# Wangshihu12/colmap-pcd

Measured on AMD Instinct MI355X. Metric: NN queries/sec + BA-iter ms, 10M-pt cloud / 1M 3D feats, higher is better.
Workload: dtype f32 (NN distances) / f64 (association, BA); 1 GPU; M: 10000000-pt 'planes' cloud / 1000000 queries + BA scene 1000 cams / 1000000 pts / 4721253 obs / 900000 lidar terms (OPENCV), the same total at every N; cloud_points=10000000, queries=1000000, queries_this_rank=1000000, parallelism=single GPU

## Files before the change

### colmap-pcd_amd/csrc/ba.hip

```cpp
#include <algorithm>
#include <cmath>

#include "ba_cam_jac.h"
#include "ba_handle.h"
#include "ba_math.h"
#include "common.h"

namespace pcd {

template <int MODEL, bool SHARED>
struct BaCam {
  static constexpr int K = cam_num_params(MODEL >= 0 ? MODEL : 0);
  int model = MODEL;
  const double* p = nullptr;
  double v[K];
  __device__ __forceinline__ void resolve(const BaDev& d, int cm) {
    if (MODEL < 0) model = d.cam_model[cm];
    p = d.cam_params + d.cam_off[cm];
  }
  __device__ __forceinline__ explicit BaCam(const BaDev& d) {
    if (!SHARED) return;
    resolve(d, d.shared_cam);
    if (MODEL >= 0) {
#pragma unroll
      for (int k = 0; k < K; ++k) v[k] = p[k];
    }
  }
  __device__ __forceinline__ const double* params() const { return (SHARED && MODEL >= 0) ? v : p; }
  __device__ __forceinline__ void of_image(const BaDev& d, int im) {
    if (!SHARED) resolve(d, d.image_cam[im]);
  }
};

__device__ __forceinline__ void load_pose(const BaDev& d, int im, double pose[7]) {
#pragma unroll
  for (int k = 0; k < 7; ++k) pose[k] = d.poses[7 * (size_t)im + k];
}
template <int MODEL, bool SHARED>
__device__ __forceinline__ void eval_block_at(const BaCam<MODEL, SHARED>& cam, const double pose[7], const double X[3],
                                              double ox, double oy, ReprojBlock& b, double q[4]) {
  double t[3];
#pragma unroll
  for (int k = 0; k < 4; ++k) q[k] = pose[k];
#pragma unroll
  for (int k = 0; k < 3; ++k) t[k] = pose[4 + k];
  reproj_eval(cam.model, cam.params(), q, t, X, ox, oy, b);
}
template <int MODEL>
__device__ __forceinline__ void eval_block(const BaDev& d, int im, const double X[3], double ox, double oy,
                                           ReprojBlock& b, double q[4]) {
  const double* pose = d.poses + 7 * (size_t)im;
  double t[3];
#pragma unroll
  for (int k = 0; k < 4; ++k) q[k] = pose[k];
#pragma unroll
  for (int k = 0; k < 3; ++k) t[k] = pose[4 + k];
  const int cm = d.image_cam[im];
  const int model = MODEL >= 0 ? MODEL : d.cam_model[cm];
  reproj_eval(model, d.cam_params + d.cam_off[cm], q, t, X, ox, oy, b);
}
__device__ __forceinline__ double wave_uniform(double v) {
  const long long u = __double_as_longlong(v);
  const unsigned lo = (unsigned)__builtin_amdgcn_readfirstlane((int)(unsigned)u);
  const unsigned hi = (unsigned)__builtin_amdgcn_readfirstlane((int)(unsigned)((unsigned long long)u >> 32));
  return __longlong_as_double((long long)(((unsigned long long)hi << 32) | lo));
}

template <int N>
__device__ __forceinline__ void wave_store_rows(double* __restrict__ out, uint64_t row0, int cnt, const double (&v)[N],
                                                double* __restrict__ lds) {
  static_assert(N % 2 == 0, "rows are moved in 16-byte units");
  const int lane = threadIdx.x & 63;
#pragma unroll
  for (int k = 0; k < N; ++k) lds[lane * N + k] = v[k];
  __builtin_amdgcn_fence(__ATOMIC_RELEASE, "workgroup");
  __builtin_amdgcn_wave_barrier();
  __builtin_amdgcn_fence(__ATOMIC_ACQUIRE, "workgroup");
  const double2* src = reinterpret_cast<const double2*>(lds);
  double2* dst = reinterpret_cast<double2*>(out + row0 * N);
  const int units = cnt * (N / 2);
#pragma unroll
  for (int j = 0; j < N / 2; ++j) {
    const int u = j * 64 + lane;
    if (u < units) dst[u] = src[u];
  }
  __builtin_amdgcn_fence(__ATOMIC_RELEASE, "workgroup");
  __builtin_amdgcn_wave_barrier();
}

template <int MODEL, bool BLOCKS, bool SHARED>
__global__ __launch_bounds__(256) void k_ba_points(BaDev d, double* __restrict__ Hpt, double* __restrict__ gpt,
                                                   double* __restrict__ cost_partial) {
  __shared__ double s_half[2][64][9];
  const int sl = threadIdx.x >> 7, half = (threadIdx.x >> 6) & 1, lane = threadIdx.x & 63;
  const int slice = blockIdx.x * 2 + sl;
  const int t = slice * 64 + lane;
  double cost = 0.0;
  double H[6] = {0, 0, 0, 0, 0, 0}, g[3] = {0, 0, 0};
  int p = -1;
  bool cpt = true;
  double X[3] = {0, 0, 0};
  BaCam<MODEL, SHARED> cam(d);
  if (slice < d.nslices) {
    p = d.pt_order[t];
    const uint32_t s0 = d.slice_start[slice], s1 = d.slice_start[slice + 1];
    if (p >= 0) {
      X[0] = d.points[3 * (size_t)p]; X[1] = d.points[3 * (size_t)p + 1]; X[2] = d.points[3 * (size_t)p + 2];
      cpt = d.point_const && d.point_const[p];
    }
    for (uint32_t s = s0 + lane + 64u * half; s < s1; s += 128) {
      const int im = d.sell_img[s];
      if (im < 0) continue;
      ReprojBlock b;
      double q[4], pose[7];
      cam.of_image(d, im);
      load_pose(d, im, pose);
      eval_block_at(cam, pose, X, d.sell_xy[2 * (size_t)s], d.sell_xy[2 * (size_t)s + 1], b, q);
      double rho0, rho1;
      loss_eval(d.loss_type, d.loss_scale, b.r[0] * b.r[0] + b.r[1] * b.r[1], rho0, rho1);
      cost += 0.5 * rho0;
      if (BLOCKS && !cpt) {
        const double sr = sqrt(rho1);
        double J[6];
#pragma unroll
        for (int r = 0; r < 2; ++r)
#pragma unroll
          for (int k = 0; k < 3; ++k)
            J[3 * r + k] = sr * (b.M[3 * r] * b.D[k] + b.M[3 * r + 1] * b.D[3 + k] + b.M[3 * r + 2] * b.D[6 + k]);
        const double r0 = sr * b.r[0], r1 = sr * b.r[1];
        H[0] += J[0] * J[0] + J[3] * J[3]; H[1] += J[0] * J[1] + J[3] * J[4]; H[2] += J[0] * J[2] + J[3] * J[5];
        H[3] += J[1] * J[1] + J[4] * J[4]; H[4] += J[1] * J[2] + J[4] * J[5]; H[5] += J[2] * J[2] + J[5] * J[5];
        g[0] += J[0] * r0 + J[3] * r1; g[1] += J[1] * r0 + J[4] * r1; g[2] += J[2] * r0 + J[5] * r1;
      }
    }
  }
  if (BLOCKS && half == 1) {
#pragma unroll
    for (int k = 0; k < 6; ++k) s_half[sl][lane][k] = H[k];
#pragma unroll
    for (int k = 0; k < 3; ++k) s_half[sl][lane][6 + k] = g[k];
  }
  __syncthreads();
  if (half == 0 && slice < d.nslices) {
    if (BLOCKS) {
#pragma unroll
      for (int k = 0; k < 6; ++k) H[k] += s_half[sl][lane][k];
#pragma unroll
      for (int k = 0; k < 3; ++k) g[k] += s_half[sl][lane][6 + k];
    }
    if (p >= 0) {
      for (uint32_t e = d.pt_lidar_start[p]; e < d.pt_lidar_start[p + 1]; ++e) {
        const uint32_t l = d.pt_lidar_list[e];
        const double abcd[4] = {d.lidar_abcd[4 * (size_t)l], d.lidar_abcd[4 * (size_t)l + 1],
                                d.lidar_abcd[4 * (size_t)l + 2], d.lidar_abcd[4 * (size_t)l + 3]};
        double r, J[3];
        lidar_eval(X, abcd, d.lidar_w[l], 0, r, J);
        double rho0, rho1;
        loss_eval(d.loss_type, d.loss_scale, r * r, rho0, rho1);
        cost += 0.5 * rho0;
        if (BLOCKS && !cpt) {
          const double sr = sqrt(rho1);
          const double rc = sr * r;
          J[0] *= sr; J[1] *= sr; J[2] *= sr;
          H[0] += J[0] * J[0]; H[1] += J[0] * J[1]; H[2] += J[0] * J[2];
          H[3] += J[1] * J[1]; H[4] += J[1] * J[2]; H[5] += J[2] * J[2];
          g[0] += J[0] * rc; g[1] += J[1] * rc; g[2] += J[2] * rc;
        }
      }
      if (BLOCKS && Hpt) {
        double* h = Hpt + 9 * (size_t)p;
        h[0] = H[0]; h[1] = H[1]; h[2] = H[2]; h[3] = H[1]; h[4] = H[3]; h[5] = H[4]; h[6] = H[2]; h[7] = H[4]; h[8] = H[5];
      }
      if (BLOCKS && gpt) { gpt[3 * (size_t)p] = g[0]; gpt[3 * (size_t)p + 1] = g[1]; gpt[3 * (size_t)p + 2] = g[2]; }
    }
  }
  __syncthreads();
  __shared__ double s_c[256];
  s_c[threadIdx.x] = cost;
  __syncthreads();
  for (int off = 128; off > 0; off >>= 1) {
    if ((int)threadIdx.x < off) s_c[threadIdx.x] += s_c[threadIdx.x + off];
    __syncthreads();
  }
  if (threadIdx.x == 0) cost_partial[blockIdx.x] = s_c[0];
}

template <int MODEL, bool SHARED>
__global__ __launch_bounds__(256) void k_ba_cost(BaDev d, double* __restrict__ cost_partial) {
  double cost = 0.0;
  BaCam<MODEL, SHARED> cam(d);
  for (uint64_t i = blockIdx.x * (uint64_t)256 + threadIdx.x; i < d.O + d.L; i += (uint64_t)gridDim.x * 256) {
    if (i < d.O) {
      const int im = d.obs_image[i], pt = d.obs_point[i];
      const double X[3] = {d.points[3 * (size_t)pt], d.points[3 * (size_t)pt + 1], d.points[3 * (size_t)pt + 2]};
      ReprojBlock b;
      double q[4];
      double pose[7];
      const int im0 = __builtin_amdgcn_readfirstlane(im);
      if (__all(im == im0)) {
#pragma unroll
        for (int k = 0; k < 7; ++k) pose[k] = wave_uniform(d.poses[7 * (size_t)im0 + k]);
      } else {
        load_pose(d, im, pose);
      }
      cam.of_image(d, im);
      eval_block_at(cam, pose, X, d.obs_xy[2 * i], d.obs_xy[2 * i + 1], b, q);
      double rho0, rho1;
      loss_eval(d.loss_type, d.loss_scale, b.r[0] * b.r[0] + b.r[1] * b.r[1], rho0, rho1);
      cost += 0.5 * rho0;
    } else {
      const uint64_t l = i - d.O;
      const int pt = d.lidar_point[l];
      const double X[3] = {d.points[3 * (size_t)pt], d.points[3 * (size_t)pt + 1], d.points[3 * (size_t)pt + 2]};
      const double abcd[4] = {d.lidar_abcd[4 * l], d.lidar_abcd[4 * l + 1], d.lidar_abcd[4 * l + 2], d.lidar_abcd[4 * l + 3]};
      double r, J[3];
      lidar_eval(X, abcd, d.lidar_w[l], 0, r, J);
      double rho0, rho1;
      loss_eval(d.loss_type, d.loss_scale, r * r, rho0, rho1);
      cost += 0.5 * rho0;
    }
  }
  __shared__ double s_c[256];
  s_c[threadIdx.x] = cost;
  __syncthreads();
  for (int off = 128; off > 0; off >>= 1) {
    if ((int)threadIdx.x < off) s_c[threadIdx.x] += s_c[threadIdx.x + off];
    __syncthreads();
  }
  if (threadIdx.x == 0) cost_partial[blockIdx.x] = s_c[0];
}
constexpr unsigned kCostBlocks = 1u << 20;

constexpr int kSumThreads = 1024;
__global__ __launch_bounds__(kSumThreads) void k_sum_partials(const double* __restrict__ partial, int n,
                                                              double* __restrict__ out) {
  constexpr int T = kSumThreads;
  __shared__ double s_c[T];
  double a[8] = {0.0, 0.0, 0.0, 0.0, 0.0, 0.0, 0.0, 0.0};
  int i = threadIdx.x;
  for (; i + 7 * T < n; i += 8 * T) {
#pragma unroll
    for (int j = 0; j < 8; ++j) a[j] += partial[i + j * T];
  }
  for (; i < n; i += T) a[0] += partial[i];
  s_c[threadIdx.x] = ((a[0] + a[1]) + (a[2] + a[3])) + ((a[4] + a[5]) + (a[6] + a[7]));
  __syncthreads();
  for (int off = T / 2; off > 0; off >>= 1) {
    if ((int)threadIdx.x < off) s_c[threadIdx.x] += s_c[threadIdx.x + off];
    __syncthreads();
  }
  if (threadIdx.x == 0) out[0] = s_c[0];
}

constexpr uint32_t kImgSeg = 1024;
constexpr int kRowColStride = 132;
static_assert(7 * kRowColStride <= 64 * 18, "the staged rows share the W transpose scratch");
typedef double mfma_f64x4 __attribute__((ext_vector_type(4)));

template <int MODEL, bool WANT_W>
__global__ __launch_bounds__(256, (MODEL == 4 && WANT_W) ? 4 : 1) void k_ba_images(BaDev d, double* __restrict__ partial,
                                                                       double* __restrict__ W_o) {
  __shared__ __attribute__((aligned(16))) double s_w[4][64 * 18];
  __shared__ double s_a[4][2][27];
  const int im = (int)d.seg_img[blockIdx.x];
  const int lane = threadIdx.x & 63;
  const int wave = __builtin_amdgcn_readfirstlane((int)(threadIdx.x >> 6));
  const bool cpose = d.image_const_pose && d.image_const_pose[im];
  mfma_f64x4 acc = {0.0, 0.0, 0.0, 0.0};
  const unsigned tmask = d.image_const_tvec ? d.image_const_tvec[im] : 0u;
  const uint32_t e_beg = d.seg_begin[blockIdx.x];
  const uint32_t e_end = min(d.seg_begin[blockIdx.x + 1], d.img_obs_start[im + 1]);
  const int op_k = lane >> 4, op_c = (lane & 7) == 7 ? 0 : (lane & 7);
  const double* op_src = s_w[wave] + op_c * kRowColStride + 2 * op_k + ((lane >> 3) & 1);
  if (!cpose || WANT_W) {
    for (uint32_t e0 = e_beg; e0 < e_end; e0 += 256) {
      const uint32_t e = e0 + threadIdx.x;
      const bool active = e < e_end;
      const int cnt = (int)min(64u, e_end > e0 + wave * 64u ? e_end - (e0 + wave * 64u) : 0u);
      double w[18];
#pragma unroll
      for (int k = 0; k < 18; ++k) w[k] = 0.0;
      double J[12], r0 = 0.0, r1 = 0.0;
#pragma unroll
      for (int k = 0; k < 12; ++k) J[k] = 0.0;
      if (active && !cpose) {
        const int pt = d.img_pt[e];
        const double X[3] = {d.points[3 * (size_t)pt], d.points[3 * (size_t)pt + 1], d.points[3 * (size_t)pt + 2]};
        ReprojBlock b;
        double q[4];
        eval_block<MODEL>(d, im, X, d.img_xy[2 * (size_t)e], d.img_xy[2 * (size_t)e + 1], b, q);
        double rho0, rho1;
        loss_eval(d.loss_type, d.loss_scale, b.r[0] * b.r[0] + b.r[1] * b.r[1], rho0, rho1);
        const double sr = sqrt(rho1);
        double Jq[8], Jt[6], JX[6], Jqt[6];
        reproj_jacobians(b, Jq, Jt, JX);
        quat_tangent(q, Jq, Jqt);
#pragma unroll
        for (int r = 0; r < 2; ++r)
#pragma unroll
          for (int k = 0; k < 3; ++k) {
            J[6 * r + k] = sr * Jqt[3 * r + k];
            J[6 * r + 3 + k] = ((tmask >> k) & 1u) ? 0.0 : sr * Jt[3 * r + k];
          }
        r0 = sr * b.r[0];
        r1 = sr * b.r[1];
        if (WANT_W && !(d.point_const && d.point_const[pt])) {
#pragma unroll
          for (int a = 0; a < 6; ++a)
#pragma unroll
            for (int c = 0; c < 3; ++c) w[3 * a + c] = J[a] * (sr * JX[c]) + J[6 + a] * (sr * JX[3 + c]);
        }
      }
      if (!cpose && cnt > 0) {
        double2* row_dst = reinterpret_cast<double2*>(s_w[wave]) + lane;
#pragma unroll
        for (int c = 0; c < 6; ++c) row_dst[c * (kRowColStride / 2)] = make_double2(J[c], J[6 + c]);
        row_dst[6 * (kRowColStride / 2)] = make_double2(r0, r1);
        __builtin_amdgcn_fence(__ATOMIC_RELEASE, "workgroup");
        __builtin_amdgcn_wave_barrier();
        __builtin_amdgcn_fence(__ATOMIC_ACQUIRE, "workgroup");
#pragma unroll
        for (int s = 0; s < 16; ++s) {
          const double a = op_src[8 * s];
          acc = __builtin_amdgcn_mfma_f64_16x16x4f64(a, a, acc, 0, 0, 0);
        }
        __builtin_amdgcn_fence(__ATOMIC_RELEASE, "workgroup");
        __builtin_amdgcn_wave_barrier();
      }
      if (WANT_W) {
        const uint32_t o = active ? d.img_obs[e] : 0u;
        const uint32_t o_first = (uint32_t)__builtin_amdgcn_readfirstlane((int)o);
        const bool contiguous = __all(!active || o == o_first + (uint32_t)lane);
        if (contiguous) {
          wave_store_rows<18>(W_o, o_first, cnt, w, s_w[wave]);
        } else if (active) {
          double* dst = W_o + 18 * (size_t)o;
#pragma unroll
          for (int k = 0; k < 18; ++k) dst[k] = w[k];
        }
      }
    }
  }
  {
    const int g = lane >> 4, h = (lane >> 3) & 1, c = lane & 7;
#pragma unroll
    for (int hi = 0; hi < 2; ++hi) {
      const int a = g + 4 * hi;
      const double v = h ? acc[2 + hi] : acc[hi];
      if (a < 6 && c >= a && c < 7) s_a[wave][h][c == 6 ? 21 + a : a * 6 - a * (a - 1) / 2 + (c - a)] = v;
    }
  }
  __syncthreads();
  if (threadIdx.x < 27) {
    const int k = threadIdx.x;
    partial[27 * (size_t)blockIdx.x + k] = ((s_a[0][0][k] + s_a[0][1][k]) + (s_a[1][0][k] + s_a[1][1][k])) +
                                           ((s_a[2][0][k] + s_a[2][1][k]) + (s_a[3][0][k] + s_a[3][1][k]));
  }
}

__global__ __launch_bounds__(64) void k_ba_images_reduce(BaDev d, const double* __restrict__ partial,
                                                         double* __restrict__ Himg, double* __restrict__ gimg) {
  const int im = blockIdx.x * 2 + (threadIdx.x >> 5), k = threadIdx.x & 31;
  if (im >= d.I || k >= 27) return;
  double v = 0.0;
  for (uint32_t sgm = d.img_seg_start[im]; sgm < d.img_seg_start[im + 1]; ++sgm) v += partial[27 * (size_t)sgm + k];
  if (k >= 21) {
    if (gimg) gimg[6 * (size_t)im + (k - 21)] = v;
  } else if (Himg) {
    int a = 0, kk = k;
    while (kk >= 6 - a) { kk -= 6 - a; ++a; }
    const int c = a + kk;
    Himg[36 * (size_t)im + 6 * a + c] = v;
    Himg[36 * (size_t)im + 6 * c + a] = v;
  }
}

__host__ __device__ constexpr int cam_ne(int K) { return K * (K + 1) / 2 + 6 * K + K; }
__host__ __device__ constexpr int cam_ent_l(int K, int e) {
  const int ncc = K * (K + 1) / 2;
  if (e < ncc) { int a = 0; while (e >= K - a) { e -= K - a; ++a; } return a; }
  e -= ncc;
  if (e < 6 * K) return e / 6;
  return e - 6 * K;
}
__host__ __device__ constexpr int cam_ent_r(int K, int e) {
  const int ncc = K * (K + 1) / 2;
  if (e < ncc) { int a = 0; while (e >= K - a) { e -= K - a; ++a; } return a + e; }
  e -= ncc;
  if (e < 6 * K) return K + e % 6;
  return K + 6;
}

template <int MODEL, int CH>
__device__ __forceinline__ void cam_accumulate(const BaDev& d, int im, double* __restrict__ partial) {
  constexpr int K = MODEL >= 0 ? cam_num_params(MODEL >= 0 ? MODEL : 0) : PCD_CAM_JAC_STRIDE;
  constexpr int NE = cam_ne(K), PER = (NE + 3) / 4, E0 = CH * PER, E1 = E0 + PER < NE ? E0 + PER : NE;
  constexpr int NA = K + 7;
  const int lane = threadIdx.x & 63;
  const bool cpose = d.image_const_pose && d.image_const_pose[im];
  const unsigned tmask = d.image_const_tvec ? d.image_const_tvec[im] : 0u;
  const int cm = d.image_cam[im];
  const double* cam = d.cam_params + d.cam_off[cm];
  const uint8_t* refine = d.cam_refine ? d.cam_refine + d.cam_off[cm] : nullptr;
  const int model = MODEL >= 0 ? MODEL : d.cam_model[cm];
  double acc[PER > 0 ? PER : 1];
#pragma unroll
  for (int t = 0; t < PER; ++t) acc[t] = 0.0;
  for (uint32_t e = d.img_obs_start[im] + lane; e < d.img_obs_start[im + 1]; e += 64) {
    const int pt = d.img_pt[e];
    const double X[3] = {d.points[3 * (size_t)pt], d.points[3 * (size_t)pt + 1], d.points[3 * (size_t)pt + 2]};
    ReprojBlock b;
    double q[4];
    eval_block<MODEL>(d, im, X, d.img_xy[2 * (size_t)e], d.img_xy[2 * (size_t)e + 1], b, q);
    double rho0, rho1;
    loss_eval(d.loss_type, d.loss_scale, b.r[0] * b.r[0] + b.r[1] * b.r[1], rho0, rho1);
    const double sr = sqrt(rho1);
    double A[2][NA];
    {
      const double* pose = d.poses + 7 * (size_t)im;
// ... 508 lines not shown
}

static void launch_points(const pcd_ba* b, const BaDev& d, double* Hpt, double* gpt, hipStream_t s) {
  PCD_BA_DISPATCH_CAM(b->uniform_model, d.shared_cam >= 0,
                      hipLaunchKernelGGL((k_ba_points<M, true, SH>), dim3(cost_blocks(b, true)), dim3(256), 0, s, d, Hpt, gpt,
                                         b->cost_partial.p));
}
static void launch_images(const pcd_ba* b, const BaDev& d, double* Himg, double* gimg, double* W, hipStream_t s) {
  if (b->nseg) {
    PCD_BA_DISPATCH(b->uniform_model,
                    if (W) hipLaunchKernelGGL((k_ba_images<M, true>), dim3(b->nseg), dim3(256), 0, s, d, b->img_partial.p, W);
                    else hipLaunchKernelGGL((k_ba_images<M, false>), dim3(b->nseg), dim3(256), 0, s, d, b->img_partial.p, W));
  }
  hipLaunchKernelGGL(k_ba_images_reduce, dim3(div_up(b->I, 2)), dim3(64), 0, s, d, b->img_partial.p, Himg, gimg);
}

pcd_status pcd::ba_normal_equations(pcd_ba* b, const uint32_t* w_order, double* Hpt, double* gpt, double* cost,
                                    double* Himg, double* gimg, double* W, hipStream_t s) {
  PCD_TRY(b->img_partial.reserve(27 * (size_t)std::max(b->nseg, 1u)));
  BaDev d = b->dev();
  launch_points(b, d, Hpt, gpt, s);
  hipLaunchKernelGGL(k_sum_partials, dim3(1), dim3(kSumThreads), 0, s, b->cost_partial.p, (int)cost_blocks(b, true), cost);
  if (w_order) d.img_obs = w_order;
  launch_images(b, d, Himg, gimg, W, s);
  return PCD_OK;
}

extern "C" {

pcd_status pcd_ba_create(const pcd_ba_desc* d, pcd_ba** out) {
  return pcd::guard([&]() -> pcd_status {
  PCD_REQUIRE(d && out, "null pointer");
  *out = nullptr;
  PCD_REQUIRE(d->num_cameras > 0 && d->cam_model && d->cam_param_offset && d->cam_params, "cameras");
  PCD_REQUIRE(d->num_images > 0 && d->poses && d->image_camera, "images");
  PCD_REQUIRE(d->num_points > 0 && d->points, "points");
  PCD_REQUIRE(d->num_obs == 0 || (d->obs_image && d->obs_point && d->obs_xy), "observations");
  PCD_REQUIRE(d->num_lidar == 0 || (d->lidar_point && d->lidar_abcd && d->lidar_weight), "lidar terms");
  PCD_REQUIRE(d->loss_type >= 0 && d->loss_type <= 2, "loss_type");
  PCD_REQUIRE(d->loss_type == PCD_LOSS_TRIVIAL || d->loss_scale > 0, "loss_scale");
  PCD_REQUIRE(d->num_obs < 0xFFFFFFF0ull && d->num_lidar < 0xFFFFFFF0ull, "too many residual blocks");
  for (int c = 0; c < d->num_cameras; ++c) {
    const int k = pcd_camera_num_params(d->cam_model[c]);
    PCD_REQUIRE(k > 0, "unknown camera model id");
    PCD_REQUIRE(d->cam_param_offset[c] >= 0 && (uint64_t)d->cam_param_offset[c] + k <= d->cam_params_len,
                "camera parameter offsets");
  }
  for (int i = 0; i < d->num_images; ++i)
    PCD_REQUIRE(d->image_camera[i] >= 0 && d->image_camera[i] < d->num_cameras, "image_camera out of range");
  for (uint64_t o = 0; o < d->num_obs; ++o) {
    PCD_REQUIRE(d->obs_image[o] >= 0 && d->obs_image[o] < d->num_images, "obs_image out of range");
    PCD_REQUIRE(d->obs_point[o] >= 0 && d->obs_point[o] < d->num_points, "obs_point out of range");
  }
  for (uint64_t l = 0; l < d->num_lidar; ++l)
    PCD_REQUIRE(d->lidar_point[l] >= 0 && d->lidar_point[l] < d->num_points, "lidar_point out of range");
  PCD_TRY(require_device(d->device));

  pcd_ba* b = new pcd_ba();
  b->device = d->device;
  b->C = d->num_cameras; b->I = d->num_images; b->P = d->num_points; b->O = d->num_obs; b->L = d->num_lidar;
  b->loss_type = d->loss_type; b->loss_scale = d->loss_scale;
  b->cam_params_len = d->cam_params_len;
  for (int c = 0; c < d->num_cameras; ++c) b->cam_stride = std::max(b->cam_stride, cam_num_params(d->cam_model[c]));
  b->uniform_model = d->cam_model[0];
  for (int c = 1; c < d->num_cameras; ++c)
    if (d->cam_model[c] != b->uniform_model) b->uniform_model = -1;
  b->shared_cam = d->image_camera[0];
  for (int i = 1; i < d->num_images; ++i)
    if (d->image_camera[i] != b->shared_cam) b->shared_cam = -1;
  auto fail = [&](pcd_status st) { pcd_ba_destroy(b); return st; };
#define UP(buf, src, n) do { pcd_status _st = upload(b->buf, src, (size_t)(n)); if (_st != PCD_OK) return fail(_st); } while (0)
  UP(cam_model, d->cam_model, b->C); UP(cam_off, d->cam_param_offset, b->C); UP(cam_params, d->cam_params, d->cam_params_len);
  UP(poses, d->poses, 7 * (size_t)b->I); UP(image_cam, d->image_camera, b->I);
  UP(points, d->points, 3 * (size_t)b->P);
  UP(obs_image, d->obs_image, b->O); UP(obs_point, d->obs_point, b->O); UP(obs_xy, d->obs_xy, 2 * b->O);
  UP(lidar_point, d->lidar_point, b->L); UP(lidar_abcd, d->lidar_abcd, 4 * b->L); UP(lidar_w, d->lidar_weight, b->L);
  if (d->image_const_pose) { b->has_cpose = true; UP(image_const_pose, d->image_const_pose, b->I); }
  if (d->image_const_tvec) { b->has_ctvec = true; UP(image_const_tvec, d->image_const_tvec, b->I); }
  if (d->point_const) { b->has_cpt = true; UP(point_const, d->point_const, b->P); }
  if (d->camera_refine) { b->has_refine = true; UP(cam_refine, d->camera_refine, d->cam_params_len); }
  for (uint64_t k = 0; d->camera_refine && k < d->cam_params_len; ++k) b->refines_intrinsics |= d->camera_refine[k] != 0;

  std::vector<uint32_t> st, li;
  build_csr(d->obs_point, b->O, b->P, st, li);
  {
    uint32_t maxlen = 0;
    for (int p = 0; p < b->P; ++p) maxlen = std::max(maxlen, st[p + 1] - st[p]);
    std::vector<uint32_t> bucket((size_t)maxlen + 2, 0);
    for (int p = 0; p < b->P; ++p) bucket[(size_t)(st[p + 1] - st[p]) + 1]++;
    for (size_t k = 1; k < bucket.size(); ++k) bucket[k] += bucket[k - 1];
    const int nslices = (b->P + 63) / 64;
    b->nslices = nslices;
    std::vector<int> order((size_t)nslices * 64, -1);
    for (int p = 0; p < b->P; ++p) order[bucket[st[p + 1] - st[p]]++] = p;
    std::vector<uint32_t> slice_start(nslices + 1, 0);
    for (int s = 0; s < nslices; ++s) {
      uint32_t mx = 0;
      for (int l = 63; l >= 0; --l) {
        const int p = order[(size_t)s * 64 + l];
        if (p >= 0) { mx = st[p + 1] - st[p]; break; }
      }
      slice_start[s + 1] = slice_start[s] + mx * 64;
    }
    const size_t nslots = slice_start[nslices];
    UP(pt_order, order.data(), order.size());
    UP(slice_start, slice_start.data(), slice_start.size());
    UP(pt_obs_start, st.data(), st.size()); UP(pt_obs_list, li.data(), li.size());
    UP(pt_lidar_start, st.data(), st.size()); UP(pt_lidar_list, li.data(), li.size());
    pcd_status sa = b->sell_img.reserve(std::max<size_t>(nslots, 1));
    if (sa == PCD_OK) sa = b->sell_xy.reserve(std::max<size_t>(2 * nslots, 2));
    if (sa != PCD_OK) return fail(sa);
    if (nslots)
      hipLaunchKernelGGL(k_ba_fill_sell, dim3(div_up((size_t)nslices * 64, 256)), dim3(256), 0, nullptr, b->pt_order.p,
                         b->slice_start.p, b->pt_lidar_start.p, b->pt_lidar_list.p, b->obs_image.p, b->obs_xy.p, nslices,
                         b->sell_img.p, b->sell_xy.p);
    if (hipDeviceSynchronize() != hipSuccess || hipGetLastError() != hipSuccess) {
      set_error("pcd_ba_create: filling the per-track layout failed");
      return fail(PCD_ERR_HIP);
    }
  }
  build_csr(d->lidar_point, b->L, b->P, st, li);
  UP(pt_lidar_start, st.data(), st.size()); UP(pt_lidar_list, li.data(), li.size());
  build_csr(d->obs_image, b->O, b->I, st, li);
  {
    UP(img_obs_start, st.data(), st.size());
    {
      std::vector<uint32_t> seg_img, seg_begin, img_seg_start(b->I + 1, 0);
      for (int i = 0; i < b->I; ++i) {
        img_seg_start[i] = (uint32_t)seg_img.size();
        for (uint32_t e = st[i]; e < st[i + 1]; e += kImgSeg) { seg_img.push_back((uint32_t)i); seg_begin.push_back(e); }
      }
      img_seg_start[b->I] = (uint32_t)seg_img.size();
      b->nseg = (uint32_t)seg_img.size();
      seg_begin.push_back((uint32_t)b->O);
      UP(seg_img, seg_img.data(), seg_img.size());
      UP(seg_begin, seg_begin.data(), seg_begin.size());
      UP(img_seg_start, img_seg_start.data(), img_seg_start.size());
    }
    {
      std::vector<uint32_t> cst, cli;
      build_csr(d->image_camera, (uint64_t)b->I, b->C, cst, cli);
      UP(cam_img_start, cst.data(), cst.size());
      UP(cam_img_list, cli.data(), cli.size());
    }
    UP(img_obs, li.data(), li.size());
    pcd_status sa = b->img_pt.reserve(std::max<size_t>(b->O, 1));
    if (sa == PCD_OK) sa = b->img_xy.reserve(std::max<size_t>(2 * b->O, 2));
    if (sa != PCD_OK) return fail(sa);
    if (b->O)
      hipLaunchKernelGGL(k_ba_fill_image_major, dim3(div_up(b->O, 256)), dim3(256), 0, nullptr, b->img_obs.p,
                         b->obs_point.p, b->obs_xy.p, b->O, b->img_pt.p, b->img_xy.p);
    if (hipDeviceSynchronize() != hipSuccess || hipGetLastError() != hipSuccess) {
      set_error("pcd_ba_create: filling the image-major layout failed");
      return fail(PCD_ERR_HIP);
    }
  }
#undef UP
  {
    b->h_pose_row.assign(b->O, 0xFFFFFFFFu);
    std::vector<uint32_t> vobs;
    vobs.reserve(b->O);
    for (uint64_t o = 0; o < b->O; ++o)
      if (!(d->image_const_pose && d->image_const_pose[d->obs_image[o]])) {
        b->h_pose_row[o] = (uint32_t)vobs.size();
        vobs.push_back((uint32_t)o);
      }
    b->n_pose_rows = vobs.size();
    if (b->n_pose_rows != b->O) {
      pcd_status sv = upload(b->vobs, vobs.data(), vobs.size());
      if (sv != PCD_OK) return fail(sv);
    }
  }
  pcd_status s1 = b->cost_partial.reserve((size_t)std::max(cost_blocks(b, true), cost_blocks(b, false)) + 1);
  if (s1 != PCD_OK) return fail(s1);
  if ((s1 = b->cost.reserve(1)) != PCD_OK) return fail(s1);
  *out = b;
  return PCD_OK;
  });
}

void pcd_ba_destroy(pcd_ba* b) {
  if (!b) return;
  (void)hipSetDevice(b->device);
  delete b;
}

pcd_status pcd_ba_set_parameters(pcd_ba* b, const double* poses, const double* points) {
  PCD_REQUIRE(b, "null handle");
  PCD_HIP_TRY(hipSetDevice(b->device));
  if (poses) PCD_HIP_TRY(hipMemcpy(b->poses.p, poses, 7 * (size_t)b->I * sizeof(double), hipMemcpyHostToDevice));
  if (points) PCD_HIP_TRY(hipMemcpy(b->points.p, points, 3 * (size_t)b->P * sizeof(double), hipMemcpyHostToDevice));
  return PCD_OK;
}

pcd_status pcd_ba_set_parameters_device(pcd_ba* b, const double* d_poses, const double* d_points, void* stream) {
  PCD_TRY(require_device(b ? b->device : 0));
  PCD_REQUIRE(b, "null handle");
  PCD_REFUSE_CAPTURE(stream);
  PCD_HIP_TRY(hipSetDevice(b->device));
  hipStream_t s = (hipStream_t)stream;
  if (d_poses && d_poses != b->poses.p)
    PCD_HIP_TRY(hipMemcpyAsync(b->poses.p, d_poses, 7 * (size_t)b->I * sizeof(double), hipMemcpyDeviceToDevice, s));
  if (d_points && d_points != b->points.p)
    PCD_HIP_TRY(hipMemcpyAsync(b->points.p, d_points, 3 * (size_t)b->P * sizeof(double), hipMemcpyDeviceToDevice, s));
  return PCD_OK;
// ... 292 lines not shown
```

### colmap-pcd_amd/csrc/ba_handle.h

```cpp
#pragma once
#include <memory>

#include "ba_cam_jac.h"
#include "common.h"

namespace pcd {

struct BaDev {
  const int* cam_model; const int* cam_off; const double* cam_params;
  const double* poses; const int* image_cam; const uint8_t* image_const_pose; const uint8_t* image_const_tvec;
  const double* points; const uint8_t* point_const;
  const int* obs_image; const int* obs_point; const double* obs_xy;
  const int* lidar_point; const double* lidar_abcd; const double* lidar_w;
  const int* pt_order;
  const uint32_t* slice_start;
  const int* sell_img;
  const double* sell_xy;
  const uint32_t* pt_lidar_start; const uint32_t* pt_lidar_list;
  const uint32_t* img_obs_start;
  const int* img_pt;
  const uint32_t* img_obs;
  const uint32_t* seg_img;
  const uint32_t* seg_begin;
  const uint32_t* img_seg_start;
  const uint8_t* cam_refine;
  const uint32_t* cam_img_start;
  const uint32_t* cam_img_list;
  int C;
  int cam_k;
  const double* img_xy;
  int I, P, nslices; uint64_t O, L;
  int loss_type; double loss_scale;
  int shared_cam;
};

struct BaSchur;
struct BaSchurDelete { void operator()(BaSchur* s) const; };

template <typename T>
static pcd_status upload(DevBuf<T>& b, const T* src, size_t n) {
  PCD_TRY(b.reserve(std::max<size_t>(n, 1)));
  if (n) PCD_HIP_TRY(hipMemcpy(b.p, src, n * sizeof(T), hipMemcpyHostToDevice));
  return PCD_OK;
}

pcd_status ba_normal_equations(pcd_ba* b, const uint32_t* w_order, double* Hpt, double* gpt, double* cost, double* Himg,
                               double* gimg, double* W, hipStream_t s);

}

struct pcd_ba {
  int device = 0;
  int C = 0, I = 0, P = 0, nslices = 0;
  uint64_t O = 0, L = 0, cam_params_len = 0;
  int loss_type = 0;
  double loss_scale = 1.0;
  int uniform_model = -1;
  int shared_cam = -1;
  pcd::DevBuf<int> cam_model, cam_off, image_cam, obs_image, obs_point, lidar_point, pt_order, sell_img, img_pt;
  pcd::DevBuf<double> cam_params, poses, points, obs_xy, lidar_abcd, lidar_w, sell_xy, img_xy;
  pcd::DevBuf<uint8_t> image_const_pose, image_const_tvec, point_const;
  bool has_cpose = false, has_ctvec = false, has_cpt = false;
  pcd::DevBuf<uint32_t> slice_start, pt_lidar_start, pt_lidar_list, img_obs_start, img_obs, cam_img_start, cam_img_list;
  pcd::DevBuf<uint32_t> seg_img, seg_begin, img_seg_start;
  uint32_t nseg = 0;
  pcd::DevBuf<double> img_partial;
  pcd::DevBuf<uint8_t> cam_refine;
  bool has_refine = false;
  pcd::DevBuf<double> cam_partial;
  pcd::DevBuf<double> cost_partial, cost;
  pcd::DevBuf<double> o_res, o_jq, o_jt, o_jx, o_jl, o_himg, o_gimg, o_hpt, o_gpt, o_w, o_jc, o_hcam, o_gcam, o_ecam, o_wcam;
  std::vector<uint32_t> h_pose_row;
  uint64_t n_pose_rows = 0;
  pcd::DevBuf<uint32_t> vobs;
  pcd::DevBuf<double> p_jq, p_jt;
  pcd::PinnedBuf<double> h_blocks;
  int cam_stride = 0;
  pcd::DevBuf<double> o_rec, p_jc;
  pcd::DevBuf<uint32_t> pt_obs_start, pt_obs_list;
  pcd::DevBuf<double> f_sq, f_depth, f_part, f_summary;
  pcd::DevBuf<uint8_t> f_u8;
  bool refines_intrinsics = false;
  std::unique_ptr<pcd::BaSchur, pcd::BaSchurDelete> schur;
  pcd::BaDev dev() const {
    pcd::BaDev d;
    d.cam_model = cam_model.p; d.cam_off = cam_off.p; d.cam_params = cam_params.p;
    d.poses = poses.p; d.image_cam = image_cam.p;
    d.image_const_pose = has_cpose ? image_const_pose.p : nullptr;
    d.image_const_tvec = has_ctvec ? image_const_tvec.p : nullptr;
    d.points = points.p; d.point_const = has_cpt ? point_const.p : nullptr;
    d.obs_image = obs_image.p; d.obs_point = obs_point.p; d.obs_xy = obs_xy.p;
    d.lidar_point = lidar_point.p; d.lidar_abcd = lidar_abcd.p; d.lidar_w = lidar_w.p;
    d.pt_order = pt_order.p; d.slice_start = slice_start.p; d.sell_img = sell_img.p; d.sell_xy = sell_xy.p;
    d.pt_lidar_start = pt_lidar_start.p; d.pt_lidar_list = pt_lidar_list.p;
    d.img_obs_start = img_obs_start.p; d.img_pt = img_pt.p; d.img_xy = img_xy.p; d.img_obs = img_obs.p;
    d.seg_img = seg_img.p; d.seg_begin = seg_begin.p; d.img_seg_start = img_seg_start.p;
    d.cam_refine = has_refine ? cam_refine.p : nullptr; d.cam_img_start = cam_img_start.p; d.cam_img_list = cam_img_list.p;
    d.C = C; d.shared_cam = shared_cam; d.cam_k = (uniform_model >= 0 && uniform_model <= 4) ? pcd::cam_num_params(uniform_model) : PCD_CAM_JAC_STRIDE;
    d.I = I; d.P = P; d.nslices = nslices; d.O = O; d.L = L; d.loss_type = loss_type; d.loss_scale = loss_scale;
    return d;
  }
};
```

Before: 781.3 million queries/s.

## Prefetch BA point/image operands and precompute first lidar term per slot

In the points kernel, the next SELL image index and the observation xy are now software-prefetched one iteration ahead. The first lidar plane for each thread slot is precomputed on the host into a coalesced SoA array, which removes the dependent CSR indirection for the common single-term case. In the image kernel, camera parameters and pose are hoisted out of the loop as wave-uniform values pinned in SGPRs, and the next point index, coordinates and const flag are prefetched across iterations. This is meant to hide gather latency in BA, at the cost of extra device buffers, more registers and inline-asm register pinning that may hurt occupancy.

```diff
diff --git a/colmap-pcd_amd/csrc/ba.hip b/colmap-pcd_amd/csrc/ba.hip
--- a/colmap-pcd_amd/csrc/ba.hip
+++ b/colmap-pcd_amd/csrc/ba.hip
@@ -66,11 +66,21 @@
   return __longlong_as_double((long long)(((unsigned long long)hi << 32) | lo));
 }
 
+__device__ __forceinline__ double sgpr_pin(double v) {
+  asm volatile("" : "+s"(v));
+  return v;
+}
+
+template <typename T>
+__device__ __forceinline__ T vgpr_pin(T v) {
+  asm volatile("" : "+v"(v));
+  return v;
+}
+
 template <int N>
 __device__ __forceinline__ void wave_store_rows(double* __restrict__ out, uint64_t row0, int cnt, const double (&v)[N],
-                                                double* __restrict__ lds) {
+                                                double* __restrict__ lds, int lane) {
   static_assert(N % 2 == 0, "rows are moved in 16-byte units");
-  const int lane = threadIdx.x & 63;
 #pragma unroll
   for (int k = 0; k < N; ++k) lds[lane * N + k] = v[k];
   __builtin_amdgcn_fence(__ATOMIC_RELEASE, "workgroup");
@@ -87,52 +97,103 @@
   __builtin_amdgcn_fence(__ATOMIC_RELEASE, "workgroup");
   __builtin_amdgcn_wave_barrier();
 }
+template <int N>
+__device__ __forceinline__ void wave_store_rows(double* __restrict__ out, uint64_t row0, int cnt, const double (&v)[N],
+                                                double* __restrict__ lds) {
+  wave_store_rows<N>(out, row0, cnt, v, lds, (int)(threadIdx.x & 63));
+}
+
+template <bool BLOCKS>
+__device__ __forceinline__ void points_add_lidar(const BaDev& d, const double X[3], const double abcd[4], double w, bool cpt,
+                                                 double& cost, double H[6], double g[3]) {
+  double r, J[3];
+  lidar_eval(X, abcd, w, 0, r, J);
+  double rho0, rho1;
+  loss_eval(d.loss_type, d.loss_scale, r * r, rho0, rho1);
+  cost += 0.5 * rho0;
+  if (BLOCKS && !cpt) {
+    const double sr = sqrt(rho1);
+    const double rc = sr * r;
+    J[0] *= sr; J[1] *= sr; J[2] *= sr;
+    H[0] += J[0] * J[0]; H[1] += J[0] * J[1]; H[2] += J[0] * J[2];
+    H[3] += J[1] * J[1]; H[4] += J[1] * J[2]; H[5] += J[2] * J[2];
+    g[0] += J[0] * rc; g[1] += J[1] * rc; g[2] += J[2] * rc;
+  }
+}
+
+__device__ __forceinline__ void load_lidar_first(const BaDev& d, int half, int t, uint32_t& ln, double lf[5]) {
+  if (half != 0 || !d.L) return;
+  const size_t ntr = 64 * (size_t)d.nslices;
+  ln = d.pt_lidar_cnt[t];
+#pragma unroll
+  for (int k = 0; k < 5; ++k) lf[k] = d.pt_lidar_first[k * ntr + t];
+}
 
 template <int MODEL, bool BLOCKS, bool SHARED>
 __global__ __launch_bounds__(256) void k_ba_points(BaDev d, double* __restrict__ Hpt, double* __restrict__ gpt,
                                                    double* __restrict__ cost_partial) {
   __shared__ double s_half[2][64][9];
-  const int sl = threadIdx.x >> 7, half = (threadIdx.x >> 6) & 1, lane = threadIdx.x & 63;
+  const int sl = __builtin_amdgcn_readfirstlane((int)(threadIdx.x >> 7));
+  const int half = __builtin_amdgcn_readfirstlane((int)((threadIdx.x >> 6) & 1));
+  const int lane = threadIdx.x & 63;
   const int slice = blockIdx.x * 2 + sl;
   const int t = slice * 64 + lane;
   double cost = 0.0;
   double H[6] = {0, 0, 0, 0, 0, 0}, g[3] = {0, 0, 0};
   int p = -1;
-  bool cpt = true;
+  unsigned cpt_b = 1;
   double X[3] = {0, 0, 0};
+  uint32_t ln = 0;
+  double lf[5] = {0, 0, 0, 0, 0};
+  constexpr bool kLidarEarly = SHARED;
   BaCam<MODEL, SHARED> cam(d);
   if (slice < d.nslices) {
+    const uint32_t s0 = d.slice_start[slice], s1 = d.slice_start[slice + 1];
+    uint32_t sb = s0 + 64u * half;
+    const uint32_t sc = sb < s1 ? sb + lane : 0u;
+    int im = d.sell_img[sc];
+    double ox = d.sell_xy[2 * (size_t)sc], oy = d.sell_xy[2 * (size_t)sc + 1];
     p = d.pt_order[t];
-    const uint32_t s0 = d.slice_start[slice], s1 = d.slice_start[slice + 1];
+    if (kLidarEarly) load_lidar_first(d, half, t, ln, lf);
     if (p >= 0) {
       X[0] = d.points[3 * (size_t)p]; X[1] = d.points[3 * (size_t)p + 1]; X[2] = d.points[3 * (size_t)p + 2];
-      cpt = d.point_const && d.point_const[p];
-    }
-    for (uint32_t s = s0 + lane + 64u * half; s < s1; s += 128) {
-      const int im = d.sell_img[s];
-      if (im < 0) continue;
-      ReprojBlock b;
-      double q[4], pose[7];
-      cam.of_image(d, im);
-      load_pose(d, im, pose);
-      eval_block_at(cam, pose, X, d.sell_xy[2 * (size_t)s], d.sell_xy[2 * (size_t)s + 1], b, q);
-      double rho0, rho1;
-      loss_eval(d.loss_type, d.loss_scale, b.r[0] * b.r[0] + b.r[1] * b.r[1], rho0, rho1);
-      cost += 0.5 * rho0;
-      if (BLOCKS && !cpt) {
-        const double sr = sqrt(rho1);
-        double J[6];
-#pragma unroll
-        for (int r = 0; r < 2; ++r)
-#pragma unroll
-          for (int k = 0; k < 3; ++k)
-            J[3 * r + k] = sr * (b.M[3 * r] * b.D[k] + b.M[3 * r + 1] * b.D[3 + k] + b.M[3 * r + 2] * b.D[6 + k]);
-        const double r0 = sr * b.r[0], r1 = sr * b.r[1];
-        H[0] += J[0] * J[0] + J[3] * J[3]; H[1] += J[0] * J[1] + J[3] * J[4]; H[2] += J[0] * J[2] + J[3] * J[5];
-        H[3] += J[1] * J[1] + J[4] * J[4]; H[4] += J[1] * J[2] + J[4] * J[5]; H[5] += J[2] * J[2] + J[5] * J[5];
-        g[0] += J[0] * r0 + J[3] * r1; g[1] += J[1] * r0 + J[4] * r1; g[2] += J[2] * r0 + J[5] * r1;
-      }
-    }
+      cpt_b = d.point_const ? d.point_const[p] : 0u;
+    }
+    while (sb < s1) {
+      const uint32_t sn = sb + 128;
+      const int im_next = d.sell_img[sn < s1 ? sn + lane : 0u];
+      if (im >= 0) {
+        ReprojBlock b;
+        double q[4], pose[7];
+        cam.of_image(d, im);
+        load_pose(d, im, pose);
+        eval_block_at(cam, pose, X, ox, oy, b, q);
+        double rho0, rho1;
+        loss_eval(d.loss_type, d.loss_scale, b.r[0] * b.r[0] + b.r[1] * b.r[1], rho0, rho1);
+        cost += 0.5 * rho0;
+        cpt_b = vgpr_pin(cpt_b);
+        if (BLOCKS && cpt_b == 0) {
+          const double sr = sqrt(rho1);
+          double J[6];
+#pragma unroll
+          for (int r = 0; r < 2; ++r)
+#pragma unroll
+            for (int k = 0; k < 3; ++k)
+              J[3 * r + k] = sr * (b.M[3 * r] * b.D[k] + b.M[3 * r + 1] * b.D[3 + k] + b.M[3 * r + 2] * b.D[6 + k]);
+          const double r0 = sr * b.r[0], r1 = sr * b.r[1];
+          H[0] += J[0] * J[0] + J[3] * J[3]; H[1] += J[0] * J[1] + J[3] * J[4]; H[2] += J[0] * J[2] + J[3] * J[5];
+          H[3] += J[1] * J[1] + J[4] * J[4]; H[4] += J[1] * J[2] + J[4] * J[5]; H[5] += J[2] * J[2] + J[5] * J[5];
+          g[0] += J[0] * r0 + J[3] * r1; g[1] += J[1] * r0 + J[4] * r1; g[2] += J[2] * r0 + J[5] * r1;
+        }
+      }
+      sb = sn;
+      im = vgpr_pin(im_next);
+      if (sb < s1) {
+        ox = d.sell_xy[2 * ((size_t)sb + lane)];
+        oy = d.sell_xy[2 * ((size_t)sb + lane) + 1];
+      }
+    }
+    if (!kLidarEarly) load_lidar_first(d, half, t, ln, lf);
   }
   if (BLOCKS && half == 1) {
 #pragma unroll
@@ -149,22 +210,14 @@
       for (int k = 0; k < 3; ++k) g[k] += s_half[sl][lane][6 + k];
     }
     if (p >= 0) {
-      for (uint32_t e = d.pt_lidar_start[p]; e < d.pt_lidar_start[p + 1]; ++e) {
-        const uint32_t l = d.pt_lidar_list[e];
-        const double abcd[4] = {d.lidar_abcd[4 * (size_t)l], d.lidar_abcd[4 * (size_t)l + 1],
-                                d.lidar_abcd[4 * (size_t)l + 2], d.lidar_abcd[4 * (size_t)l + 3]};
-        double r, J[3];
-        lidar_eval(X, abcd, d.lidar_w[l], 0, r, J);
-        double rho0, rho1;
-        loss_eval(d.loss_type, d.loss_scale, r * r, rho0, rho1);
-        cost += 0.5 * rho0;
-        if (BLOCKS && !cpt) {
-          const double sr = sqrt(rho1);
-          const double rc = sr * r;
-          J[0] *= sr; J[1] *= sr; J[2] *= sr;
-          H[0] += J[0] * J[0]; H[1] += J[0] * J[1]; H[2] += J[0] * J[2];
-          H[3] += J[1] * J[1]; H[4] += J[1] * J[2]; H[5] += J[2] * J[2];
-          g[0] += J[0] * rc; g[1] += J[1] * rc; g[2] += J[2] * rc;
+      if (ln) {
+        points_add_lidar<BLOCKS>(d, X, lf, lf[4], cpt_b != 0, cost, H, g);
+        const uint32_t le = ln > 1 ? d.pt_lidar_start[p] : 0u;
+        for (uint32_t e = le + 1; e < le + ln; ++e) {
+          const uint32_t l = d.pt_lidar_list[e];
+          const double abcd[4] = {d.lidar_abcd[4 * (size_t)l], d.lidar_abcd[4 * (size_t)l + 1],
+                                  d.lidar_abcd[4 * (size_t)l + 2], d.lidar_abcd[4 * (size_t)l + 3]};
+          points_add_lidar<BLOCKS>(d, X, abcd, d.lidar_w[l], cpt_b != 0, cost, H, g);
         }
       }
       if (BLOCKS && Hpt) {
@@ -257,6 +310,25 @@
 static_assert(7 * kRowColStride <= 64 * 18, "the staged rows share the W transpose scratch");
 typedef double mfma_f64x4 __attribute__((ext_vector_type(4)));
 
+template <int MODEL>
+struct BaImageCam {
+  static constexpr int K = MODEL >= 0 ? cam_num_params(MODEL >= 0 ? MODEL : 0) : PCD_CAM_JAC_STRIDE;
+  int model = MODEL;
+  double v[K];
+  __device__ __forceinline__ BaImageCam(const BaDev& d, int im) {
+    const int cm = d.image_cam[im];
+    if (MODEL < 0) model = d.cam_model[cm];
+    const double* p = d.cam_params + d.cam_off[cm];
+    const int kn = MODEL >= 0 ? K : cam_num_params(model);
+#pragma unroll
+    for (int k = 0; k < K; ++k) v[k] = wave_uniform(p[k < kn ? k : 0]);
+  }
+};
+
+__device__ __forceinline__ const uint8_t* const_byte(const BaDev& d, bool has_pc, uint32_t pt) {
+  return has_pc ? d.point_const + pt : reinterpret_cast<const uint8_t*>(d.points + 3 * (size_t)pt);
+}
+
 template <int MODEL, bool WANT_W>
 __global__ __launch_bounds__(256, (MODEL == 4 && WANT_W) ? 4 : 1) void k_ba_images(BaDev d, double* __restrict__ partial,
                                                                        double* __restrict__ W_o) {
@@ -265,18 +337,49 @@
   const int im = (int)d.seg_img[blockIdx.x];
   const int lane = threadIdx.x & 63;
   const int wave = __builtin_amdgcn_readfirstlane((int)(threadIdx.x >> 6));
-  const bool cpose = d.image_const_pose && d.image_const_pose[im];
+  const uint8_t* any_byte = reinterpret_cast<const uint8_t*>(d.seg_img + blockIdx.x);
+  const unsigned cpose_b = *(d.image_const_pose ? d.image_const_pose + im : any_byte);
+  const unsigned tmask_b = *(d.image_const_tvec ? d.image_const_tvec + im : any_byte);
   mfma_f64x4 acc = {0.0, 0.0, 0.0, 0.0};
-  const unsigned tmask = d.image_const_tvec ? d.image_const_tvec[im] : 0u;
   const uint32_t e_beg = d.seg_begin[blockIdx.x];
   const uint32_t e_end = min(d.seg_begin[blockIdx.x + 1], d.img_obs_start[im + 1]);
+  BaImageCam<MODEL> cam(d, im);
+  double q[4], tv[3];
+#pragma unroll
+  for (int k = 0; k < 4; ++k) q[k] = wave_uniform(d.poses[7 * (size_t)im + k]);
+#pragma unroll
+  for (int k = 0; k < 3; ++k) tv[k] = wave_uniform(d.poses[7 * (size_t)im + 4 + k]);
   const int op_k = lane >> 4, op_c = (lane & 7) == 7 ? 0 : (lane & 7);
   const double* op_src = s_w[wave] + op_c * kRowColStride + 2 * op_k + ((lane >> 3) & 1);
+  const bool cpose = d.image_const_pose && cpose_b;
+  const unsigned tmask = d.image_const_tvec ? tmask_b : 0u;
   if (!cpose || WANT_W) {
+    const uint32_t e_last = e_end - 1;
+    const bool has_pc = WANT_W && d.point_const;
+    uint32_t pt = 0, o = 0, pc = 0;
+    double ox = 0.0, oy = 0.0, X[3] = {0.0, 0.0, 0.0};
+    {
+      const uint32_t ec = min(e_beg + threadIdx.x, e_last);
+      pt = (uint32_t)d.img_pt[ec]; ox = d.img_xy[2 * (size_t)ec]; oy = d.img_xy[2 * (size_t)ec + 1];
+      if (WANT_W) o = d.img_obs[ec];
+      X[0] = d.points[3 * (size_t)pt]; X[1] = d.points[3 * (size_t)pt + 1]; X[2] = d.points[3 * (size_t)pt + 2];
+      if (WANT_W) pc = *const_byte(d, has_pc, pt);
+    }
     for (uint32_t e0 = e_beg; e0 < e_end; e0 += 256) {
       const uint32_t e = e0 + threadIdx.x;
       const bool active = e < e_end;
       const int cnt = (int)min(64u, e_end > e0 + wave * 64u ? e_end - (e0 + wave * 64u) : 0u);
+#pragma unroll
+      for (int k = 0; k < 4; ++k) q[k] = sgpr_pin(q[k]);
+#pragma unroll
+      for (int k = 0; k < 3; ++k) tv[k] = sgpr_pin(tv[k]);
+#pragma unroll
+      for (int k = 0; k < BaImageCam<MODEL>::K; ++k) cam.v[k] = sgpr_pin(cam.v[k]);
+      const uint32_t en = (e_last >= 256u && e <= e_last - 256u) ? e + 256u : e_last;
+      uint32_t pt_n = 0, o_n = 0;
+      double ox_n = 0.0, oy_n = 0.0;
+      pt_n = (uint32_t)d.img_pt[en]; ox_n = d.img_xy[2 * (size_t)en]; oy_n = d.img_xy[2 * (size_t)en + 1];
+      if (WANT_W) o_n = d.img_obs[en];
       double w[18];
 #pragma unroll
       for (int k = 0; k < 18; ++k) w[k] = 0.0;
@@ -284,11 +387,8 @@
 #pragma unroll
       for (int k = 0; k < 12; ++k) J[k] = 0.0;
       if (active && !cpose) {
-        const int pt = d.img_pt[e];
-        const double X[3] = {d.points[3 * (size_t)pt], d.points[3 * (size_t)pt + 1], d.points[3 * (size_t)pt + 2]};
         ReprojBlock b;
-        double q[4];
-        eval_block<MODEL>(d, im, X, d.img_xy[2 * (size_t)e], d.img_xy[2 * (size_t)e + 1], b, q);
+        reproj_eval(cam.model, cam.v, q, tv, X, ox, oy, b);
         double rho0, rho1;
         loss_eval(d.loss_type, d.loss_scale, b.r[0] * b.r[0] + b.r[1] * b.r[1], rho0, rho1);
         const double sr = sqrt(rho1);
@@ -304,15 +404,22 @@
           }
         r0 = sr * b.r[0];
         r1 = sr * b.r[1];
-        if (WANT_W && !(d.point_const && d.point_const[pt])) {
+        if (WANT_W && !(has_pc && pc != 0)) {
 #pragma unroll
           for (int a = 0; a < 6; ++a)
 #pragma unroll
             for (int c = 0; c < 3; ++c) w[3 * a + c] = J[a] * (sr * JX[c]) + J[6 + a] * (sr * JX[3 + c]);
         }
       }
+      {
+        X[0] = d.points[3 * (size_t)pt_n]; X[1] = d.points[3 * (size_t)pt_n + 1]; X[2] = d.points[3 * (size_t)pt_n + 2];
+        if (WANT_W) pc = *const_byte(d, has_pc, pt_n);
+        ox = vgpr_pin(ox_n);
+        oy = vgpr_pin(oy_n);
+      }
+      const int lane_i = vgpr_pin(lane);
       if (!cpose && cnt > 0) {
-        double2* row_dst = reinterpret_cast<double2*>(s_w[wave]) + lane;
+        double2* row_dst = reinterpret_cast<double2*>(s_w[wave]) + lane_i;
 #pragma unroll
         for (int c = 0; c < 6; ++c) row_dst[c * (kRowColStride / 2)] = make_double2(J[c], J[6 + c]);
         row_dst[6 * (kRowColStride / 2)] = make_double2(r0, r1);
@@ -328,13 +435,14 @@
         __builtin_amdgcn_wave_barrier();
       }
       if (WANT_W) {
-        const uint32_t o = active ? d.img_obs[e] : 0u;
-        const uint32_t o_first = (uint32_t)__builtin_amdgcn_readfirstlane((int)o);
-        const bool contiguous = __all(!active || o == o_first + (uint32_t)lane);
+        const uint32_t oa = active ? o : 0u;
+        o = vgpr_pin(o_n);
+        const uint32_t o_first = (uint32_t)__builtin_amdgcn_readfirstlane((int)oa);
+        const bool contiguous = __all(!active || oa == o_first + (uint32_t)lane_i);
         if (contiguous) {
-          wave_store_rows<18>(W_o, o_first, cnt, w, s_w[wave]);
+          wave_store_rows<18>(W_o, o_first, cnt, w, s_w[wave], lane_i);
         } else if (active) {
-          double* dst = W_o + 18 * (size_t)o;
+          double* dst = W_o + 18 * (size_t)oa;
 #pragma unroll
           for (int k = 0; k < 18; ++k) dst[k] = w[k];
         }
@@ -1009,6 +1117,7 @@
   for (uint64_t k = 0; d->camera_refine && k < d->cam_params_len; ++k) b->refines_intrinsics |= d->camera_refine[k] != 0;
 
   std::vector<uint32_t> st, li;
+  std::vector<int> order;
   build_csr(d->obs_point, b->O, b->P, st, li);
   {
     uint32_t maxlen = 0;
@@ -1018,7 +1127,7 @@
     for (size_t k = 1; k < bucket.size(); ++k) bucket[k] += bucket[k - 1];
     const int nslices = (b->P + 63) / 64;
     b->nslices = nslices;
-    std::vector<int> order((size_t)nslices * 64, -1);
+    order.assign((size_t)nslices * 64, -1);
     for (int p = 0; p < b->P; ++p) order[bucket[st[p + 1] - st[p]]++] = p;
     std::vector<uint32_t> slice_start(nslices + 1, 0);
     for (int s = 0; s < nslices; ++s) {
@@ -1048,6 +1157,21 @@
   }
   build_csr(d->lidar_point, b->L, b->P, st, li);
   UP(pt_lidar_start, st.data(), st.size()); UP(pt_lidar_list, li.data(), li.size());
+  if (b->L) {
+    const size_t ntr = order.size();
+    std::vector<double> first(5 * ntr, 0.0);
+    std::vector<uint32_t> cnt(ntr, 0);
+    for (size_t t = 0; t < ntr; ++t) {
+      const int p = order[t];
+      if (p < 0 || st[p] == st[p + 1]) continue;
+      cnt[t] = st[p + 1] - st[p];
+      const uint32_t l = li[st[p]];
+      for (int k = 0; k < 4; ++k) first[k * ntr + t] = d->lidar_abcd[4 * (size_t)l + k];
+      first[4 * ntr + t] = d->lidar_weight[l];
+    }
+    UP(pt_lidar_first, first.data(), first.size());
+    UP(pt_lidar_cnt, cnt.data(), cnt.size());
+  }
   build_csr(d->obs_image, b->O, b->I, st, li);
   {
     UP(img_obs_start, st.data(), st.size());
diff --git a/colmap-pcd_amd/csrc/ba_handle.h b/colmap-pcd_amd/csrc/ba_handle.h
--- a/colmap-pcd_amd/csrc/ba_handle.h
+++ b/colmap-pcd_amd/csrc/ba_handle.h
@@ -17,6 +17,8 @@
   const int* sell_img;
   const double* sell_xy;
   const uint32_t* pt_lidar_start; const uint32_t* pt_lidar_list;
+  const uint32_t* pt_lidar_cnt;
+  const double* pt_lidar_first;
   const uint32_t* img_obs_start;
   const int* img_pt;
   const uint32_t* img_obs;
@@ -58,11 +60,11 @@
   int uniform_model = -1;
   int shared_cam = -1;
   pcd::DevBuf<int> cam_model, cam_off, image_cam, obs_image, obs_point, lidar_point, pt_order, sell_img, img_pt;
-  pcd::DevBuf<double> cam_params, poses, points, obs_xy, lidar_abcd, lidar_w, sell_xy, img_xy;
+  pcd::DevBuf<double> cam_params, poses, points, obs_xy, lidar_abcd, lidar_w, sell_xy, img_xy, pt_lidar_first;
   pcd::DevBuf<uint8_t> image_const_pose, image_const_tvec, point_const;
   bool has_cpose = false, has_ctvec = false, has_cpt = false;
   pcd::DevBuf<uint32_t> slice_start, pt_lidar_start, pt_lidar_list, img_obs_start, img_obs, cam_img_start, cam_img_list;
-  pcd::DevBuf<uint32_t> seg_img, seg_begin, img_seg_start;
+  pcd::DevBuf<uint32_t> seg_img, seg_begin, img_seg_start, pt_lidar_cnt;
   uint32_t nseg = 0;
   pcd::DevBuf<double> img_partial;
   pcd::DevBuf<uint8_t> cam_refine;
@@ -93,6 +95,7 @@
     d.lidar_point = lidar_point.p; d.lidar_abcd = lidar_abcd.p; d.lidar_w = lidar_w.p;
     d.pt_order = pt_order.p; d.slice_start = slice_start.p; d.sell_img = sell_img.p; d.sell_xy = sell_xy.p;
     d.pt_lidar_start = pt_lidar_start.p; d.pt_lidar_list = pt_lidar_list.p;
+    d.pt_lidar_first = L ? pt_lidar_first.p : nullptr; d.pt_lidar_cnt = L ? pt_lidar_cnt.p : nullptr;
     d.img_obs_start = img_obs_start.p; d.img_pt = img_pt.p; d.img_xy = img_xy.p; d.img_obs = img_obs.p;
     d.seg_img = seg_img.p; d.seg_begin = seg_begin.p; d.img_seg_start = img_seg_start.p;
     d.cam_refine = has_refine ? cam_refine.p : nullptr; d.cam_img_start = cam_img_start.p; d.cam_img_list = cam_img_list.p;
```

New measurement: 793.0 million queries/s (median of 6 runs). 1.5% higher.
